# zerchen/AlignSDF

Measured on AMD Instinct MI355X. Metric: meshes_per_sec_hand_plus_obj_N256, higher is better.
Workload: dtype f32-class: 2 x f16 planes per operand (22 bit), 3 f16 MFMAs per product sum, f32 accumulate, every voxel <= 1e-5

## Files before the change

alignsdf_amd/csrc/sdf_mlp_f16w_kernel.h:

```cpp
#pragma once
#include "sdf_mlp_f16_kernel.h"

namespace asdf {

static_assert(ASDF16_STAGE_KB == 16, "the W form is written for the 32 KiB stages of the split-half kernel");

#define ASDF_MFMA16W(a, b, c) __builtin_amdgcn_mfma_f32_16x16x32_f16((a), (b), (c), 0, 0, 0)
#define ASDF_MFMA4W(a, b, c) __builtin_amdgcn_mfma_f32_16x16x4f32((a), (b), (c), 0, 0, 0)

__device__ __forceinline__ f32x4 acc_get4(const f32x16& a, int o) {
  f32x4 v;
  v[0] = a[o]; v[1] = a[o + 1]; v[2] = a[o + 2]; v[3] = a[o + 3];
  return v;
}
__device__ __forceinline__ void acc_set4(f32x16& a, int o, const f32x4& v) { a[o] = v[0]; a[o + 1] = v[1]; a[o + 2] = v[2]; a[o + 3] = v[3]; }

__device__ __forceinline__ f32x16 load_bias16w(const float* tile_words, int lane) {
  const int q = lane >> 4;
  const float* w0 = tile_words + (q & 1) * 16 + 4 * (q >> 1);
  int dup = 0;
  asm volatile("" : "+v"(dup));
  const float* w1 = w0 + dup;
  f32x16 r;
  acc_set4(r, 0, *reinterpret_cast<const f32x4*>(w0)); acc_set4(r, 4, *reinterpret_cast<const f32x4*>(w0 + 8));
  acc_set4(r, 8, *reinterpret_cast<const f32x4*>(w1)); acc_set4(r, 12, *reinterpret_cast<const f32x4*>(w1 + 8));
  return r;
}

__device__ __forceinline__ void pin_acc_w(f32x16& acc) {
#pragma unroll
  for (int o = 0; o < 16; o += 4) {
    f32x4 q;
    q[0] = acc[o]; q[1] = acc[o + 1]; q[2] = acc[o + 2]; q[3] = acc[o + 3];
    asm volatile("" : "+a"(q));
    acc[o] = q[0]; acc[o + 1] = q[1]; acc[o + 2] = q[2]; acc[o + 3] = q[3];
  }
}

#ifndef ASDF16_W_M0_CLOBBER
#define ASDF16_W_M0_CLOBBER 1
#endif
template <int P>
__device__ __forceinline__ void dma_piece_w(const float* src, unsigned dst) {
#if ASDF16_W_M0_CLOBBER
  asm volatile(
      "s_mov_b32 m0, %1\n\t"
      "s_nop 0\n\t"
      "global_load_lds_dwordx4 %0, off offset:%c2"
      :
      : "v"(src + (P >> 2) * 1024), "s"(dst + (P >> 2) * 4096), "i"((P & 3) * 1024)
      : "memory", "m0");
#else
  dma_piece<P>(src, dst);
#endif
}

template <int KB, int Q, int SLOT, int ABL, class Pre, class Epi>
__device__ __forceinline__ void stage16w(f32x16& acc, const h8 (&xh)[KB], const h8 (&xl)[KB], const float* ring, const float* next_src,
                                         unsigned lds_ring_base, int lane, int wave, h8 (&ah)[S16<2>::kPrefetch], h8 (&al)[S16<2>::kPrefetch],
                                         Pre&& pre, Epi&& epi) {
  using SG = S16<2>;
  constexpr int PF = SG::kPrefetch;
  constexpr int BKB = kBarrierKb;
  constexpr int nslot = (SLOT + kRing - 1) % kRing;
  static_assert(KB == 32 || KB == 16, "records per tile");
  static_assert(kS16Kb - BKB >= SG::kPieces, "one LDS-DMA piece per record behind the barrier");
  const float* src = next_src + wave * SG::kWaveFloats + lane * 4;
  const unsigned dst = lds_ring_base + (nslot * SG::kFloats + wave * SG::kWaveFloats) * 4;
  const h8* cur = reinterpret_cast<const h8*>(ring + SLOT * SG::kFloats) + lane;
  const h8* nxt = reinterpret_cast<const h8*>(ring + ((SLOT + 1) % kRing) * SG::kFloats) + lane;
  h8 bufh[kS16Kb + PF], bufl[kS16Kb + PF];
#pragma unroll
  for (int i = 0; i < PF; ++i) { bufh[i] = ah[i]; bufl[i] = al[i]; }
#pragma unroll
  for (int kb = 0; kb < kS16Kb; ++kb) {
    if (kb == BKB && !(ABL & 1)) {
      asm volatile("s_waitcnt vmcnt(8)" ::: "memory");
      if (!(ABL & 16)) __builtin_amdgcn_s_barrier();
    }
    bufh[kb + PF] = kb + PF < kS16Kb ? cur[((kb + PF) * 2 + 0) * 64] : nxt[((kb + PF - kS16Kb) * 2 + 0) * 64];
    bufl[kb + PF] = kb + PF < kS16Kb ? cur[((kb + PF) * 2 + 1) * 64] : nxt[((kb + PF - kS16Kb) * 2 + 1) * 64];
    pre(kb);
    __builtin_amdgcn_sched_barrier(0);
    const int ri = Q * kS16Kb + kb;
    const int xb = KB == 32 ? 2 * (ri % 16) : (ri & ~1), o = (KB == 32 ? ri / 16 : (ri & 1)) * 4;
    const bool snake = ri & 1;
    const int xa = xb + (snake ? 1 : 0), xc = xb + (snake ? 0 : 1);
#pragma unroll
    for (int j = 0; j < 3; ++j) {
      f32x4 s0 = acc_get4(acc, o), s1 = acc_get4(acc, 8 + o);
      f32x4& sa = snake ? s1 : s0;
      f32x4& sb = snake ? s0 : s1;
      if (j == 0) { sa = ASDF_MFMA16W(bufh[kb], xl[xa], sa); sa = ASDF_MFMA16W(bufl[kb], xh[xa], sa); }
      if (j == 1) { sa = ASDF_MFMA16W(bufh[kb], xh[xa], sa); sb = ASDF_MFMA16W(bufh[kb], xl[xc], sb); }
      if (j == 2) { sb = ASDF_MFMA16W(bufl[kb], xh[xc], sb); sb = ASDF_MFMA16W(bufh[kb], xh[xc], sb); }
      acc_set4(acc, o, s0); acc_set4(acc, 8 + o, s1);
      const int m = j == 2 ? kb - BKB : -1;
      if (!(ABL & 1) && !(ABL & 32) && m >= 0 && m < SG::kPieces) {
        if (m == 0) dma_piece_w<0>(src, dst);
        else if (m == 1) dma_piece_w<1>(src, dst);
        else if (m == 2) dma_piece_w<2>(src, dst);
        else if (m == 3) dma_piece_w<3>(src, dst);
        else if (m == 4) dma_piece_w<4>(src, dst);
        else if (m == 5) dma_piece_w<5>(src, dst);
        else if (m == 6) dma_piece_w<6>(src, dst);
        else dma_piece_w<7>(src, dst);
        __builtin_amdgcn_sched_barrier(0);
      }
      epi(kb, j);
      __builtin_amdgcn_sched_barrier(0);
    }
    __builtin_amdgcn_sched_barrier(0);
  }
#pragma unroll
  for (int i = 0; i < PF; ++i) { ah[i] = bufh[kS16Kb + i]; al[i] = bufl[kS16Kb + i]; }
}

template <int ABL = 0, bool SUB = false>
__device__ __forceinline__ void sdf_mlp_f16w_body(const DecodeParams& p) {
  using CL = CstLayout<2>;
  using SG = S16<2>;
  static_assert(lds_bytes_f16(2, 2) <= 160 * 1024, "LDS budget");
  extern __shared__ __attribute__((aligned(16))) float smem[];
  float* ring = smem;
  float* cst = smem + SG::kRingFloats;

  const int tid = threadIdx.x;
  const int lane = tid & 63;
  const int wave = __builtin_amdgcn_readfirstlane(tid >> 6);
  const int half = lane >> 5;

  float lat_vs = p.vs, lat_o0 = p.o0, lat_o1 = p.o1, lat_o2 = p.o2;
  if (p.lattice) { lat_o0 = p.lattice[0]; lat_o1 = p.lattice[1]; lat_o2 = p.lattice[2]; lat_vs = p.lattice[3]; }
  long long npts = p.P;
  if (SUB) { const long long c = *p.count_dev; npts = c < npts ? c : npts; }
  const long long ntiles = (npts + kWgPts - 1) / kWgPts;
  if ((long long)blockIdx.x >= ntiles) return;

  const unsigned lds_ring_base = (unsigned)(size_t)(__attribute__((address_space(3))) float*)ring;
  if (!SUB && p.status && p.mode != kPointList && blockIdx.x == 0 && tid == 0) reinterpret_cast<long long*>(p.status + ASDF_STATUS_CLOCK)[0] = clock64();

#pragma unroll 1
  for (int slot = 0; slot < p.num_mlps; ++slot) {
    const int head = p.first_mlp + slot;
    const float* hc = cst;
    int* wrec = reinterpret_cast<int*>(cst + CL::kFloats) + wave * kWrecInts;
    if (lane < kWrecInts) wrec[lane] = lane >= 16 ? 0 : ((lane & 7) < 3 ? 0x7fffffff : ((lane & 7) < 6 ? -1 : 0));
    asm volatile("s_waitcnt vmcnt(0)" ::: "memory");
    __syncthreads();
    {
      const f32x4* src4 = reinterpret_cast<const f32x4*>(p.cst + (size_t)head * CL::kFloats);
      for (int i = tid; i < CL::kFloats / 4; i += 256) reinterpret_cast<f32x4*>(cst)[i] = src4[i];
    }
    const float* sbase0 = p.stream + (size_t)kStagesAll * kStageFloats + (size_t)head * kS16Head * SG::kFloats;
#pragma unroll
    for (int s = 0; s < ((ABL & 33) ? kRing : kRing - 1); ++s) {
      const float* src = sbase0 + (size_t)s * SG::kFloats + wave * SG::kWaveFloats + lane * 4;
      const unsigned dst = lds_ring_base + (s * SG::kFloats + wave * SG::kWaveFloats) * 4;
#pragma unroll
      for (int c = 0; c < SG::kPieces; ++c) lds_dma16(src + c * 256, dst + c * 1024);
    }
    if (ABL & 33) asm volatile("s_waitcnt vmcnt(0)" ::: "memory");
    asm volatile("s_waitcnt vmcnt(16)" ::: "memory");
    __syncthreads();
    h8 ah[SG::kPrefetch], al[SG::kPrefetch];
#pragma unroll
    for (int i = 0; i < SG::kPrefetch; ++i) {
      ah[i] = (reinterpret_cast<const h8*>(ring) + lane)[(i * 2 + 0) * 64];
      al[i] = (reinterpret_cast<const h8*>(ring) + lane)[(i * 2 + 1) * 64];
    }
    const float mul1 = hc[CL::kB4 + 2], mul2 = hc[CL::kB4 + 3], mul0 = hc[CL::kB4 + 4];
    int audit_from = 0x7fffffff;
    if (SUB && p.audit) audit_from = p.audit_from ? *p.audit_from : 0;
    auto bias_at = [&](int off, int t) -> f32x16 { return load_bias16w(hc + off + t * 32, lane); };
    auto pt_word = [&](int off, int t, int fh) -> float {
      return hc[off + (t * 2 + (lane >> 5)) * 64 + ((lane >> 4) & 1) * 32 + 16 * fh + (lane & 15)];
    };

#pragma unroll 1
    for (long long tile = blockIdx.x; tile < ntiles; tile += gridDim.x) {
      const long long pi = tile * kWgPts + wave * kWavePts + (lane & 31);
      const bool valid = pi < npts;
      const long long po = SUB ? (valid ? (long long)p.idx[pi] : 0) : pi;
      float x0 = 0.f, x1 = 0.f, x2 = 0.f;
      if (SUB) {
        grid_point(po, p.N, p.grid_mode, lat_vs, lat_o0, lat_o1, lat_o2, x0, x1, x2);
      } else if (p.mode == kPointList) {
        if (valid) { x0 = p.xyz[pi * 3 + 0]; x1 = p.xyz[pi * 3 + 1]; x2 = p.xyz[pi * 3 + 2]; }
      } else {
        grid_point(valid ? pi : 0, p.N, p.mode, lat_vs, lat_o0, lat_o1, lat_o2, x0, x1, x2);
      }
      float amax = 0.0f, amax1 = 0.0f, amax2 = 0.0f;
      float bq[2];
      {
        const int q = lane >> 4;
#pragma unroll
        for (int g = 0; g < 2; ++g) {
          const int src = (lane & 15) + 16 * g;
          const float c0 = __shfl(x0, src), c1 = __shfl(x1, src), c2 = __shfl(x2, src);
          bq[g] = q == 0 ? c0 : q == 1 ? c1 : q == 2 ? c2 : 0.0f;
        }
      }
      auto pt_mfma = [&](f32x16& a, const float* af) {
#pragma unroll
        for (int fh = 0; fh < 2; ++fh)
#pragma unroll
          for (int g = 0; g < 2; ++g) acc_set4(a, 8 * g + 4 * fh, ASDF_MFMA4W(af[fh], bq[g], acc_get4(a, 8 * g + 4 * fh)));
      };
      const float* sbase = sbase0;
      asm volatile("" : "+s"(sbase));
      auto src_of = [&](int s) -> const float* {
        return sbase + (size_t)(s < kS16Head ? s : s - kS16Head) * SG::kFloats;
      };

      f32x16 acc1[2], acc2[2], acc3[2];
      float pf2[2];
      float w4c[2], w4n[2];
      static_assert(kPreKb >= kEpiShift + kEpiChunks, "preload K-block inside the epilogue slots");
      auto load_pf2 = [&](int t) { pf2[0] = pt_word(CL::kA2, t, 0); pf2[1] = pt_word(CL::kA2, t, 1); };
      auto load_w4 = [&](int t, int c) {
        const int wq = lane >> 4;
        const float* w4 = hc + CL::kW4 + (t * 2 + (wq & 1)) * 16 + 4 * (2 * ((c >> 1) & 1) + (wq >> 1)) + 2 * (c & 1);
        w4n[0] = w4[0]; w4n[1] = w4[1];
      };
      auto next_w4 = [&]() { w4c[0] = w4n[0]; w4c[1] = w4n[1]; };

      h8 h0h[2 * kTilesHidden], h0l[2 * kTilesHidden];
      f32x16 acc0[2];
      float pf0[2][2];
      auto l0_load = [&](int t) {
        acc0[t & 1] = bias_at(CL::kC0, t);
        pf0[t & 1][0] = pt_word(CL::kA0, t, 0); pf0[t & 1][1] = pt_word(CL::kA0, t, 1);
      };
      constexpr int kL0Front = kS16Kb / 2;
      l0_load(0);
      acc1[0] = bias_at(CL::kB1, 0);
#pragma unroll
      for (int t = 0; t < kL0Front; ++t) {
        l0_load(t + 1);
        __builtin_amdgcn_sched_barrier(0);
        f32x16 acc = acc0[t & 1];
        pt_mfma(acc, pf0[t & 1]);
        split_tile<2, 1, true>(acc, acc, mul0, h0h[2 * t], h0l[2 * t], h0h[2 * t + 1], h0l[2 * t + 1], amax);
        __builtin_amdgcn_sched_barrier(0);
      }

#define ASDF_STAGE16W(KB, Q, SLOT, ACC, XH, XL, SIDX, PRE, EPI) \
  stage16w<KB, Q, SLOT, ABL>(ACC, XH, XL, ring, src_of((SIDX) + 3), lds_ring_base, lane, wave, ah, al, PRE, EPI)

      float er[2] = {0.0f, 0.0f};
      h8 h1h[2 * kTilesL1], h1l[2 * kTilesL1];
      if (ABL & 4) for (int t = 0; t < 2 * kTilesL1; ++t) { h1h[t] = h0h[t]; h1l[t] = h0l[t]; }
#pragma unroll
      for (int t = 0; t < kTilesL1; ++t) {
        f32x16& acc = acc1[t & 1];
        auto pre = [&](int kb) {
          const int c = kb - kEpiShift;
          if (t == 0 && c >= 0 && c + 1 < kEpiChunks) l0_load(kL0Front + c + 1);
        };
        auto epi = [&](int kb, int g) {
          const int c = kb - kEpiShift;
          if (c < 0 || c >= kEpiChunks) return;
          if (t == 0) {
            const int T = kL0Front + c;
            if (g == 0) pt_mfma(acc0[T & 1], pf0[T & 1]);
#pragma unroll
            for (int e = 0; e < 8; ++e)
              if (e / 3 == g) split_part<2, 1, true>(acc0[T & 1], acc0[T & 1], mul0, h0h[2 * T], h0l[2 * T], h0h[2 * T + 1], h0l[2 * T + 1], amax, e);
            return;
          }
          if (ABL & 4) { asm volatile("" :: "v"(acc1[(t - 1) & 1])); return; }
          if (g == 0) pin_acc_w(acc1[(t - 1) & 1]);
          split_part<2, 1, true>(acc1[(t - 1) & 1], acc1[(t - 1) & 1], mul1, h1h[2 * (t - 1)], h1l[2 * (t - 1)], h1h[2 * (t - 1) + 1],
                                 h1l[2 * (t - 1) + 1], amax1, c, -1, g, er);
        };
        auto pre_last = [&](int c) {
          if (c != kPreKb) return;
          if (t + 1 < kTilesL1) acc1[(t + 1) & 1] = bias_at(CL::kB1, t + 1);
          else { acc2[0] = bias_at(CL::kC2, 0); load_pf2(0); }
        };
        if (t & 1) {
          ASDF_STAGE16W(32, 0, 2, acc, h0h, h0l, t * 2 + 0, pre, epi);
          ASDF_STAGE16W(32, 1, 3, acc, h0h, h0l, t * 2 + 1, pre_last, NoOp16());
        } else {
          ASDF_STAGE16W(32, 0, 0, acc, h0h, h0l, t * 2 + 0, pre, epi);
          ASDF_STAGE16W(32, 1, 1, acc, h0h, h0l, t * 2 + 1, pre_last, NoOp16());
        }
      }

      h8 h2h[2 * kTilesHidden], h2l[2 * kTilesHidden];
      if (ABL & 4) for (int t = 0; t < 2 * kTilesHidden; ++t) { h2h[t] = h0h[t]; h2l[t] = h0l[t]; }
      auto l2_tile = [&](int t, auto slot_tag) {
        constexpr int SLOT = decltype(slot_tag)::value;
        f32x16& acc = acc2[t & 1];
        pt_mfma(acc, pf2);
        auto epi = [&](int kb, int g) {
          const int c = kb - kEpiShift;
          if (c < 0 || c >= kEpiChunks) return;
          if (ABL & 4) { asm volatile("" :: "v"(acc2[(t + 1) & 1]), "v"(acc1[1])); return; }
          if (t > 0) {
            if (g == 0) pin_acc_w(acc2[(t - 1) & 1]);
            split_part<2, 1, true>(acc2[(t - 1) & 1], acc2[(t - 1) & 1], mul2, h2h[2 * (t - 1)], h2l[2 * (t - 1)], h2h[2 * (t - 1) + 1],
                                   h2l[2 * (t - 1) + 1], amax2, c, -1, g, er);
          } else {
            if (g == 0) pin_acc_w(acc1[(kTilesL1 - 1) & 1]);
            split_part<2, 1, true>(acc1[(kTilesL1 - 1) & 1], acc1[(kTilesL1 - 1) & 1], mul1, h1h[2 * kTilesL1 - 2], h1l[2 * kTilesL1 - 2],
                                   h1h[2 * kTilesL1 - 1], h1l[2 * kTilesL1 - 1], amax1, c, -1, g, er);
          }
        };
        auto pre_last = [&](int c) {
          if (c != kPreKb) return;
          if (t + 1 < kTilesHidden) { acc2[(t + 1) & 1] = bias_at(CL::kC2, t + 1); load_pf2(t + 1); }
          else acc3[0] = bias_at(CL::kB3, 0);
        };
        constexpr int S0 = 256 / kS16Kb;
        ASDF_STAGE16W(16, 0, SLOT, acc, h1h, h1l, S0 + t, pre_last, epi);
      };
#pragma unroll
      for (int tt = 0; tt < kTilesHidden / 4; ++tt) {
        l2_tile(4 * tt + 0, std::integral_constant<int, 0>());
        l2_tile(4 * tt + 1, std::integral_constant<int, 1>());
        l2_tile(4 * tt + 2, std::integral_constant<int, 2>());
        l2_tile(4 * tt + 3, std::integral_constant<int, 3>());
      }

      float part = 0.0f, partg = 0.0f;
      auto dot_w4_part = [&](const f32x16& a, int c, int only = -1) {
#pragma unroll
        for (int r = 0; r < 2; ++r) {
          if (only >= 0 && only != r) continue;
          const float v = __int_as_float(max(__float_as_int(a[2 * c + r]), 0));
          if (c < 4) part = fmaf(v, w4c[r], part);
          else partg = fmaf(v, w4c[r], partg);
        }
      };
#pragma unroll
      for (int t = 0; t < kTilesHidden; ++t) {
        f32x16& acc = acc3[t & 1];
        auto pre = [&](int kb) {
          const int c = kb - kEpiShift;
          if (t > 0 && c >= 0 && c + 1 < kEpiChunks) load_w4(t - 1, c + 1);
        };
        auto epi = [&](int kb, int g) {
          const int c = kb - kEpiShift;
          if (c < 0 || c >= kEpiChunks) return;
          if (ABL & 4) { asm volatile("" :: "v"(acc3[(t + 1) & 1]), "v"(acc2[1])); return; }
          if (t > 0) {
            if (g == 0) pin_acc_w(acc3[(t - 1) & 1]);
            if (g < 2) dot_w4_part(acc3[(t - 1) & 1], c, g);
            else next_w4();
          } else {
            if (g == 0) pin_acc_w(acc2[(kTilesHidden - 1) & 1]);
            split_part<2, 1, true>(acc2[(kTilesHidden - 1) & 1], acc2[(kTilesHidden - 1) & 1], mul2, h2h[2 * kTilesHidden - 2],
                                   h2l[2 * kTilesHidden - 2], h2h[2 * kTilesHidden - 1], h2l[2 * kTilesHidden - 1], amax2, c, -1, g, er);
          }
        };
        auto pre_last = [&](int c) {
          if (c != kPreKb) return;
          if (t + 1 < kTilesHidden) acc3[(t + 1) & 1] = bias_at(CL::kB3, t + 1);
          load_w4(t, 0);
          next_w4();
        };
        constexpr int S0 = 512 / kS16Kb;
        if (t & 1) {
          ASDF_STAGE16W(32, 0, 2, acc, h2h, h2l, S0 + t * 2 + 0, pre, epi);
          ASDF_STAGE16W(32, 1, 3, acc, h2h, h2l, S0 + t * 2 + 1, pre_last, NoOp16());
        } else {
          ASDF_STAGE16W(32, 0, 0, acc, h2h, h2l, S0 + t * 2 + 0, pre, epi);
          ASDF_STAGE16W(32, 1, 1, acc, h2h, h2l, S0 + t * 2 + 1, pre_last, NoOp16());
        }
      }
#pragma unroll
      for (int c = 0; c < kEpiChunks; ++c) {
        if (c + 1 < kEpiChunks) load_w4(kTilesHidden - 1, c + 1);
        dot_w4_part(acc3[(kTilesHidden - 1) & 1], c);
        next_w4();
      }
#undef ASDF_STAGE16W
      part += __shfl_xor(part, 16); partg += __shfl_xor(partg, 16);
      part += __shfl_xor(part, 32); partg += __shfl_xor(partg, 32);
      part = (lane & 16) ? partg : part;
      const float pre = part + hc[CL::kB4];
      const float sdf = tanhf(pre);
      const bool is_hand = head == 0;
      if (SUB) {
        int dm = 0, da = 0, flips = 0, na = 0;
        float sq = 0.0f;
        if (valid && half == 0) {
          const bool aud = p.audit && pi >= (long long)audit_from;
          float* out = is_hand ? p.sdf0 : p.sdf1;
          if (out) {
            const float before = out[po];
            const int d = __float_as_int(fabsf(sdf - before));
            if (aud) { da = max(da, d); flips += ((before < 0.0f) != (sdf < 0.0f)) ? 1 : 0; ++na; sq += (sdf - before) * (sdf - before); }
            else dm = max(dm, d);
            if (!aud || p.audit_from) out[po] = sdf;
          }
        }
#pragma unroll
        for (int m = 32; m >= 1; m >>= 1) {
          dm = max(dm, __shfl_xor(dm, m)); da = max(da, __shfl_xor(da, m));
          flips += __shfl_xor(flips, m); na += __shfl_xor(na, m);
          if (p.audit) sq += __shfl_xor(sq, m);
        }
        if (lane == 0) {
          if (p.status && dm) atomicMax(p.status + ASDF_STATUS_MAX_ERR, dm);
          if (p.audit && na) {
            atomicMax(p.audit + kAuditMaxErr, da); if (flips) atomicAdd(p.audit + kAuditFlips, flips); atomicAdd(p.audit + kAuditEvals, na);
            atomicAdd(reinterpret_cast<float*>(p.audit + kAuditSumSq), sq);
          }
        }
      } else if (valid && half == 0) {
        float* out = is_hand ? p.sdf0 : p.sdf1;
        if (out) out[po] = sdf;
      }
      amax *= mul0; amax1 *= mul1; amax2 *= mul2;
      const bool act_over = !(fmaxf(amax, fmaxf(amax1, amax2)) < 65504.0f);
      const int bad = (valid && (act_over || !(fabsf(sdf) <= 1.0f))) ? 1 : 0;
      if (p.status) {
        const int m0 = wave_max_i32(valid ? __float_as_int(amax) : 0), m1 = wave_max_i32(valid ? __float_as_int(amax1) : 0),
                  m2 = wave_max_i32(valid ? __float_as_int(amax2) : 0);
        if (lane == 0) { wrec[16] = max(wrec[16], m0); wrec[17] = max(wrec[17], m1); wrec[18] = max(wrec[18], m2); }
      }
      if (!SUB && p.bbox && p.mode != kPointList) {
        const bool neg = valid && half == 0 && sdf < p.neg_thr;
        int extra = bad;
        if (__any(neg || extra != 0)) {
          int i0, i1, i2;
          lattice_ijk(pi, p.N, i0, i1, i2);
          int a0 = neg ? i0 : 0x7fffffff, a1 = neg ? i1 : 0x7fffffff, a2 = neg ? i2 : 0x7fffffff;
          int b0 = neg ? i0 : -1, b1 = neg ? i1 : -1, b2 = neg ? i2 : -1, n = neg ? 1 : 0;
#pragma unroll
          for (int m = 32; m >= 1; m >>= 1) {
            a0 = min(a0, __shfl_xor(a0, m)); a1 = min(a1, __shfl_xor(a1, m)); a2 = min(a2, __shfl_xor(a2, m));
            b0 = max(b0, __shfl_xor(b0, m)); b1 = max(b1, __shfl_xor(b1, m)); b2 = max(b2, __shfl_xor(b2, m));
            n += __shfl_xor(n, m);
            extra += __shfl_xor(extra, m);
          }
          if (lane == 0 && (n | extra)) {
            wrec[0] = min(wrec[0], a0); wrec[1] = min(wrec[1], a1); wrec[2] = min(wrec[2], a2);
            wrec[3] = max(wrec[3], b0); wrec[4] = max(wrec[4], b1); wrec[5] = max(wrec[5], b2);
            wrec[6] += n; wrec[7] += extra;
          }
        }
      } else {
        const unsigned long long m = __ballot(bad);
        if (m && lane == 0) wrec[7] += __popcll(m);
      }
    }

    if (lane == 0) {
      if (p.bbox && p.mode != kPointList) {
        int* out = p.bbox + (head == 0 ? 0 : ASDF_BOX_STRIDE);
        if (wrec[6]) {
          atomicMin(out + ASDF_BOX_MIN + 0, wrec[0]); atomicMin(out + ASDF_BOX_MIN + 1, wrec[1]); atomicMin(out + ASDF_BOX_MIN + 2, wrec[2]);
          atomicMax(out + ASDF_BOX_MAX + 0, wrec[3]); atomicMax(out + ASDF_BOX_MAX + 1, wrec[4]); atomicMax(out + ASDF_BOX_MAX + 2, wrec[5]);
          atomicAdd(out + ASDF_BOX_COUNT, wrec[6]);
        }
        if (wrec[7]) atomicAdd(p.bbox + (head == 0 ? ASDF_BOX_RANGE : ASDF_BOX_STRIDE + ASDF_BOX_RANGE), wrec[7]);
      }
      if (p.status) {
        if (wrec[7]) atomicAdd(p.status + ASDF_STATUS_RANGE, wrec[7]);
        int* peak = p.status + ASDF_STATUS_PEAK + ASDF_STATUS_PEAK_STRIDE * head;
        atomicMax(peak + 0, wrec[16]); atomicMax(peak + 1, wrec[17]); atomicMax(peak + 2, wrec[18]);
      }
    }
  }
  asm volatile("s_waitcnt vmcnt(0)" ::: "memory");
  if (!SUB && p.status && p.mode != kPointList && blockIdx.x == 0 && tid == 0) reinterpret_cast<long long*>(p.status + ASDF_STATUS_CLOCK)[1] = clock64();
}


}
```

Before: 14.05.

## Interleave epilogue split steps one per MFMA and add explicit LDS waitcnts

```diff
diff --git a/alignsdf_amd/csrc/sdf_mlp_f16w_kernel.h b/alignsdf_amd/csrc/sdf_mlp_f16w_kernel.h
--- a/alignsdf_amd/csrc/sdf_mlp_f16w_kernel.h
+++ b/alignsdf_amd/csrc/sdf_mlp_f16w_kernel.h
@@ -27,14 +27,13 @@
   return r;
 }
 
-__device__ __forceinline__ void pin_acc_w(f32x16& acc) {
-#pragma unroll
-  for (int o = 0; o < 16; o += 4) {
-    f32x4 q;
-    q[0] = acc[o]; q[1] = acc[o + 1]; q[2] = acc[o + 2]; q[3] = acc[o + 3];
-    asm volatile("" : "+a"(q));
-    acc[o] = q[0]; acc[o + 1] = q[1]; acc[o + 2] = q[2]; acc[o + 3] = q[3];
-  }
+__device__ __forceinline__ float relu_acc_w(f32x16& acc, int i) {
+  const int o = i & ~3;
+  f32x4 q;
+  q[0] = acc[o]; q[1] = acc[o + 1]; q[2] = acc[o + 2]; q[3] = acc[o + 3];
+  asm volatile("" : "+a"(q));
+  acc[o] = q[0]; acc[o + 1] = q[1]; acc[o + 2] = q[2]; acc[o + 3] = q[3];
+  return __int_as_float(max(__float_as_int(acc[i]), 0));
 }
 
 #ifndef ASDF16_W_M0_CLOBBER
@@ -55,6 +54,61 @@
 #endif
 }
 
+__device__ __forceinline__ void split_step_w(f32x16& acc, float mul, h8& hi0, h8& lo0, h8& hi1, h8& lo1, float& amax, int e, int step,
+                                             float* rr) {
+  if (step == 0) { rr[0] = relu_acc_w(acc, e); return; }
+  if (step == 1) { rr[1] = relu_acc_w(acc, 8 + e); return; }
+  if (step == 4) { asm("v_max3_f32 %0, %0, %1, %2" : "+v"(amax) : "v"(rr[0]), "v"(rr[1])); return; }
+  if (step != 2 && step != 3) return;
+  const float r0 = rr[0], r1 = rr[1];
+  u32x4 H0 = __builtin_bit_cast(u32x4, hi0), L0 = __builtin_bit_cast(u32x4, lo0);
+  u32x4 H1 = __builtin_bit_cast(u32x4, hi1), L1 = __builtin_bit_cast(u32x4, lo1);
+  unsigned a = H0[e >> 1], b = L0[e >> 1], c = H1[e >> 1], d = L1[e >> 1];
+  if (step == 2) {
+    if (e & 1)
+      asm("v_fma_mixhi_f16 %0, %2, %4, 0\n\t"
+          "v_fma_mixhi_f16 %1, %3, %4, 0"
+          : "+v"(a), "+v"(c) : "v"(r0), "v"(r1), "v"(mul));
+    else
+      asm("v_fma_mixlo_f16 %0, %2, %4, 0\n\t"
+          "v_fma_mixlo_f16 %1, %3, %4, 0"
+          : "=&v"(a), "=&v"(c) : "v"(r0), "v"(r1), "v"(mul));
+    H0[e >> 1] = a; H1[e >> 1] = c;
+    hi0 = __builtin_bit_cast(h8, H0); hi1 = __builtin_bit_cast(h8, H1);
+  } else {
+    if (e & 1)
+      asm("v_fma_mixhi_f16 %0, %2, %4, -%5 op_sel:[0,0,1] op_sel_hi:[0,0,1]\n\t"
+          "v_fma_mixhi_f16 %1, %3, %4, -%6 op_sel:[0,0,1] op_sel_hi:[0,0,1]"
+          : "+v"(b), "+v"(d) : "v"(r0), "v"(r1), "v"(mul), "v"(a), "v"(c));
+    else
+      asm("v_fma_mixlo_f16 %0, %2, %4, -%5 op_sel_hi:[0,0,1]\n\t"
+          "v_fma_mixlo_f16 %1, %3, %4, -%6 op_sel_hi:[0,0,1]"
+          : "=&v"(b), "=&v"(d) : "v"(r0), "v"(r1), "v"(mul), "v"(a), "v"(c));
+    L0[e >> 1] = b; L1[e >> 1] = d;
+    lo0 = __builtin_bit_cast(h8, L0); lo1 = __builtin_bit_cast(h8, L1);
+  }
+}
+
+__device__ __forceinline__ void wait_lds_w(int n) {
+  switch (n) {
+    case 2: __builtin_amdgcn_s_waitcnt(0xc27f); break;
+    case 3: __builtin_amdgcn_s_waitcnt(0xc37f); break;
+    case 4: __builtin_amdgcn_s_waitcnt(0xc47f); break;
+    case 5: __builtin_amdgcn_s_waitcnt(0xc57f); break;
+    case 6: __builtin_amdgcn_s_waitcnt(0xc67f); break;
+    case 7: __builtin_amdgcn_s_waitcnt(0xc77f); break;
+    case 8: __builtin_amdgcn_s_waitcnt(0xc87f); break;
+    default: break;
+  }
+}
+
+#ifndef ASDF16_W_STAMPS
+struct StageStamps16w {
+  __device__ __forceinline__ void at(int) {}
+  __device__ __forceinline__ void flush(int) {}
+};
+#endif
+
 template <int KB, int Q, int SLOT, int ABL, class Pre, class Epi>
 __device__ __forceinline__ void stage16w(f32x16& acc, const h8 (&xh)[KB], const h8 (&xl)[KB], const float* ring, const float* next_src,
                                          unsigned lds_ring_base, int lane, int wave, h8 (&ah)[S16<2>::kPrefetch], h8 (&al)[S16<2>::kPrefetch],
@@ -72,30 +126,37 @@
   h8 bufh[kS16Kb + PF], bufl[kS16Kb + PF];
 #pragma unroll
   for (int i = 0; i < PF; ++i) { bufh[i] = ah[i]; bufl[i] = al[i]; }
+  StageStamps16w stamps;
 #pragma unroll
   for (int kb = 0; kb < kS16Kb; ++kb) {
+    stamps.at(kb);
     if (kb == BKB && !(ABL & 1)) {
       asm volatile("s_waitcnt vmcnt(8)" ::: "memory");
       if (!(ABL & 16)) __builtin_amdgcn_s_barrier();
     }
     bufh[kb + PF] = kb + PF < kS16Kb ? cur[((kb + PF) * 2 + 0) * 64] : nxt[((kb + PF - kS16Kb) * 2 + 0) * 64];
     bufl[kb + PF] = kb + PF < kS16Kb ? cur[((kb + PF) * 2 + 1) * 64] : nxt[((kb + PF - kS16Kb) * 2 + 1) * 64];
-    pre(kb);
+    const int pre_reads = pre(kb);
     __builtin_amdgcn_sched_barrier(0);
+    wait_lds_w(2 + pre_reads);
     const int ri = Q * kS16Kb + kb;
     const int xb = KB == 32 ? 2 * (ri % 16) : (ri & ~1), o = (KB == 32 ? ri / 16 : (ri & 1)) * 4;
     const bool snake = ri & 1;
     const int xa = xb + (snake ? 1 : 0), xc = xb + (snake ? 0 : 1);
 #pragma unroll
-    for (int j = 0; j < 3; ++j) {
+    for (int j = 0; j < 6; ++j) {
       f32x4 s0 = acc_get4(acc, o), s1 = acc_get4(acc, 8 + o);
       f32x4& sa = snake ? s1 : s0;
       f32x4& sb = snake ? s0 : s1;
-      if (j == 0) { sa = ASDF_MFMA16W(bufh[kb], xl[xa], sa); sa = ASDF_MFMA16W(bufl[kb], xh[xa], sa); }
-      if (j == 1) { sa = ASDF_MFMA16W(bufh[kb], xh[xa], sa); sb = ASDF_MFMA16W(bufh[kb], xl[xc], sb); }
-      if (j == 2) { sb = ASDF_MFMA16W(bufl[kb], xh[xc], sb); sb = ASDF_MFMA16W(bufh[kb], xh[xc], sb); }
+      if (j == 0) sa = ASDF_MFMA16W(bufh[kb], xl[xa], sa);
+      if (j == 1) sa = ASDF_MFMA16W(bufl[kb], xh[xa], sa);
+      if (j == 2) sa = ASDF_MFMA16W(bufh[kb], xh[xa], sa);
+      if (j == 3) sb = ASDF_MFMA16W(bufh[kb], xl[xc], sb);
+      if (j == 4) sb = ASDF_MFMA16W(bufl[kb], xh[xc], sb);
+      if (j == 5) sb = ASDF_MFMA16W(bufh[kb], xh[xc], sb);
       acc_set4(acc, o, s0); acc_set4(acc, 8 + o, s1);
-      const int m = j == 2 ? kb - BKB : -1;
+      __builtin_amdgcn_sched_barrier(0);
+      const int m = j == 4 ? kb - BKB : -1;
       if (!(ABL & 1) && !(ABL & 32) && m >= 0 && m < SG::kPieces) {
         if (m == 0) dma_piece_w<0>(src, dst);
         else if (m == 1) dma_piece_w<1>(src, dst);
@@ -112,6 +173,8 @@
     }
     __builtin_amdgcn_sched_barrier(0);
   }
+  stamps.at(kS16Kb);
+  stamps.flush(KB == 16 ? 2 : Q);
 #pragma unroll
   for (int i = 0; i < PF; ++i) { ah[i] = bufh[kS16Kb + i]; al[i] = bufl[kS16Kb + i]; }
 }
@@ -254,9 +317,10 @@
 #pragma unroll
       for (int t = 0; t < kTilesL1; ++t) {
         f32x16& acc = acc1[t & 1];
-        auto pre = [&](int kb) {
+        auto pre = [&](int kb) -> int {
           const int c = kb - kEpiShift;
-          if (t == 0 && c >= 0 && c + 1 < kEpiChunks) l0_load(kL0Front + c + 1);
+          if (t == 0 && c >= 0 && c + 1 < kEpiChunks) { l0_load(kL0Front + c + 1); return 6; }
+          return 0;
         };
         auto epi = [&](int kb, int g) {
           const int c = kb - kEpiShift;
@@ -266,18 +330,18 @@
             if (g == 0) pt_mfma(acc0[T & 1], pf0[T & 1]);
 #pragma unroll
             for (int e = 0; e < 8; ++e)
-              if (e / 3 == g) split_part<2, 1, true>(acc0[T & 1], acc0[T & 1], mul0, h0h[2 * T], h0l[2 * T], h0h[2 * T + 1], h0l[2 * T + 1], amax, e);
+              if ((e < 6 ? 1 + e / 2 : e - 2) == g)
+                split_part<2, 1, true>(acc0[T & 1], acc0[T & 1], mul0, h0h[2 * T], h0l[2 * T], h0h[2 * T + 1], h0l[2 * T + 1], amax, e);
             return;
           }
           if (ABL & 4) { asm volatile("" :: "v"(acc1[(t - 1) & 1])); return; }
-          if (g == 0) pin_acc_w(acc1[(t - 1) & 1]);
-          split_part<2, 1, true>(acc1[(t - 1) & 1], acc1[(t - 1) & 1], mul1, h1h[2 * (t - 1)], h1l[2 * (t - 1)], h1h[2 * (t - 1) + 1],
-                                 h1l[2 * (t - 1) + 1], amax1, c, -1, g, er);
-        };
-        auto pre_last = [&](int c) {
-          if (c != kPreKb) return;
-          if (t + 1 < kTilesL1) acc1[(t + 1) & 1] = bias_at(CL::kB1, t + 1);
-          else { acc2[0] = bias_at(CL::kC2, 0); load_pf2(0); }
+          split_step_w(acc1[(t - 1) & 1], mul1, h1h[2 * (t - 1)], h1l[2 * (t - 1)], h1h[2 * (t - 1) + 1], h1l[2 * (t - 1) + 1], amax1, c, g, er);
+        };
+        auto pre_last = [&](int c) -> int {
+          if (c != kPreKb) return 0;
+          if (t + 1 < kTilesL1) { acc1[(t + 1) & 1] = bias_at(CL::kB1, t + 1); return 4; }
+          acc2[0] = bias_at(CL::kC2, 0); load_pf2(0);
+          return 6;
         };
         if (t & 1) {
           ASDF_STAGE16W(32, 0, 2, acc, h0h, h0l, t * 2 + 0, pre, epi);
@@ -299,19 +363,17 @@
           if (c < 0 || c >= kEpiChunks) return;
           if (ABL & 4) { asm volatile("" :: "v"(acc2[(t + 1) & 1]), "v"(acc1[1])); return; }
           if (t > 0) {
-            if (g == 0) pin_acc_w(acc2[(t - 1) & 1]);
-            split_part<2, 1, true>(acc2[(t - 1) & 1], acc2[(t - 1) & 1], mul2, h2h[2 * (t - 1)], h2l[2 * (t - 1)], h2h[2 * (t - 1) + 1],
-                                   h2l[2 * (t - 1) + 1], amax2, c, -1, g, er);
+            split_step_w(acc2[(t - 1) & 1], mul2, h2h[2 * (t - 1)], h2l[2 * (t - 1)], h2h[2 * (t - 1) + 1], h2l[2 * (t - 1) + 1], amax2, c, g, er);
           } else {
-            if (g == 0) pin_acc_w(acc1[(kTilesL1 - 1) & 1]);
-            split_part<2, 1, true>(acc1[(kTilesL1 - 1) & 1], acc1[(kTilesL1 - 1) & 1], mul1, h1h[2 * kTilesL1 - 2], h1l[2 * kTilesL1 - 2],
-                                   h1h[2 * kTilesL1 - 1], h1l[2 * kTilesL1 - 1], amax1, c, -1, g, er);
-          }
-        };
-        auto pre_last = [&](int c) {
-          if (c != kPreKb) return;
-          if (t + 1 < kTilesHidden) { acc2[(t + 1) & 1] = bias_at(CL::kC2, t + 1); load_pf2(t + 1); }
-          else acc3[0] = bias_at(CL::kB3, 0);
+            split_step_w(acc1[(kTilesL1 - 1) & 1], mul1, h1h[2 * kTilesL1 - 2], h1l[2 * kTilesL1 - 2], h1h[2 * kTilesL1 - 1], h1l[2 * kTilesL1 - 1],
+                         amax1, c, g, er);
+          }
+        };
+        auto pre_last = [&](int c) -> int {
+          if (c != kPreKb) return 0;
+          if (t + 1 < kTilesHidden) { acc2[(t + 1) & 1] = bias_at(CL::kC2, t + 1); load_pf2(t + 1); return 6; }
+          acc3[0] = bias_at(CL::kB3, 0);
+          return 4;
         };
         constexpr int S0 = 256 / kS16Kb;
         ASDF_STAGE16W(16, 0, SLOT, acc, h1h, h1l, S0 + t, pre_last, epi);
@@ -334,32 +396,38 @@
           else partg = fmaf(v, w4c[r], partg);
         }
       };
+      auto dot_w4_step = [&](f32x16& a, int c, int step) {
+        const int r = step >> 1;
+        if (!(step & 1)) er[r] = relu_acc_w(a, 2 * c + r);
+        else if (c < 4) part = fmaf(er[r], w4c[r], part);
+        else partg = fmaf(er[r], w4c[r], partg);
+      };
 #pragma unroll
       for (int t = 0; t < kTilesHidden; ++t) {
         f32x16& acc = acc3[t & 1];
-        auto pre = [&](int kb) {
+        auto pre = [&](int kb) -> int {
           const int c = kb - kEpiShift;
-          if (t > 0 && c >= 0 && c + 1 < kEpiChunks) load_w4(t - 1, c + 1);
+          if (t > 0 && c >= 0 && c + 1 < kEpiChunks) { load_w4(t - 1, c + 1); return 1; }
+          return 0;
         };
         auto epi = [&](int kb, int g) {
           const int c = kb - kEpiShift;
           if (c < 0 || c >= kEpiChunks) return;
           if (ABL & 4) { asm volatile("" :: "v"(acc3[(t + 1) & 1]), "v"(acc2[1])); return; }
           if (t > 0) {
-            if (g == 0) pin_acc_w(acc3[(t - 1) & 1]);
-            if (g < 2) dot_w4_part(acc3[(t - 1) & 1], c, g);
-            else next_w4();
+            if (g < 4) dot_w4_step(acc3[(t - 1) & 1], c, g);
+            else if (g == 4) next_w4();
           } else {
-            if (g == 0) pin_acc_w(acc2[(kTilesHidden - 1) & 1]);
-            split_part<2, 1, true>(acc2[(kTilesHidden - 1) & 1], acc2[(kTilesHidden - 1) & 1], mul2, h2h[2 * kTilesHidden - 2],
-                                   h2l[2 * kTilesHidden - 2], h2h[2 * kTilesHidden - 1], h2l[2 * kTilesHidden - 1], amax2, c, -1, g, er);
-          }
-        };
-        auto pre_last = [&](int c) {
-          if (c != kPreKb) return;
+            split_step_w(acc2[(kTilesHidden - 1) & 1], mul2, h2h[2 * kTilesHidden - 2], h2l[2 * kTilesHidden - 2], h2h[2 * kTilesHidden - 1],
+                         h2l[2 * kTilesHidden - 1], amax2, c, g, er);
+          }
+        };
+        auto pre_last = [&](int c) -> int {
+          if (c != kPreKb) return 0;
           if (t + 1 < kTilesHidden) acc3[(t + 1) & 1] = bias_at(CL::kB3, t + 1);
           load_w4(t, 0);
           next_w4();
+          return t + 1 < kTilesHidden ? 5 : 1;
         };
         constexpr int S0 = 512 / kS16Kb;
         if (t & 1) {
```

New measurement: 14.23, median of 6. 1.3% higher.
